# codebits1001/CET-driven-simulation-for-3D-printing-AM-KMC-Approach

Hardware: AMD Instinct MI355X
Metric: kmc_events_per_sec (higher is better)
Workload: dtype f64

## Files before the change

### cet-driven-simulation-for-3d-printing-am-kmc-approach_amd/csrc/kernels.hpp

```cpp
#pragma once
#include "voxel.hpp"
#include "../../include/cetkmc.h"

namespace cetkmc {

struct BlockEnt { double sum; int64_t cnt; };

struct StepState {
    int64_t cur;
    int32_t status;
    int32_t pad0;
    int64_t np_pos;
    int64_t nuc_count;
    double  total;
    int64_t n_events;
    int64_t n_dep;
    double  min_margin;
};

template <class S> __device__ __forceinline__ const auto& ens_rep(unsigned r, const S& sel) { return sel.reps[r]; }
template <class S> __device__ __forceinline__ int ens_rel(const S& sel) { return sel.rel; }
template <class S> __device__ __forceinline__ unsigned ens_nz(const S& sel) { return (unsigned)sel.nz; }
template <class S> __device__ __forceinline__ int64_t ens_stride(const S& sel) { return sel.stride; }
template <class S> __device__ __forceinline__ const long long* ens_offs(const S& sel) { return sel.offs; }
// ... 832 lines not shown
    }
    const int lp = L - 1 - S.gi0;
    if (lp >= 0 && lp < S.nloc)
        for (int64_t idx = gtid; idx < (int64_t)L * L; idx += nthr) {
            const int j = (int)(idx / L), k = (int)(idx - (int64_t)j * L);
            S.dep_val[(int64_t)j * S.pitchT + k] = dep_rate(P, pymax(S.T[S.tidx(lp + 2, j, k)], 1.0));
        }
}

__global__ __launch_bounds__(64) void k_plane_reduce(SlabView S, BlockEnt* __restrict__ blocks,
                                                     const StepState* __restrict__ ss)
{
    if (ss && ss->status) return;
    const int b = blockIdx.x;
    plane_reduce_wave<false>(S.rowsum, S.rowcnt, blocks, S.L, S.Pk, S.gi0, b / 3, b % 3, (int)threadIdx.x);
}

__host__ __device__ __forceinline__ uint64_t mix64(uint64_t x)
{
    x ^= x >> 30; x *= 0xBF58476D1CE4E5B9ULL;
    x ^= x >> 27; x *= 0x94D049BB133111EBULL;
    x ^= x >> 31;
    return x;
}
__host__ __device__ __forceinline__ double counter_uniform(uint64_t seed, uint64_t step, uint64_t site)
{
    uint64_t x = mix64(seed + 0x9E3779B97F4A7C15ULL * (step + 1));
    x = mix64(x ^ (site * 0xD6E8FEB86659FD93ULL + 0x2545F4914F6CDD1DULL));
    return (double)(x >> 11) * (1.0 / 9007199254740992.0);
}
constexpr uint64_t KEY_PICK = 1ull << 40, KEY_THETA = 2ull << 40, KEY_PHI = 3ull << 40, KEY_DEFECT = 4ull << 40,
                   KEY_ACCEPT = 5ull << 40, KEY_DT = 6ull << 40;
__device__ __forceinline__ int dep_species(const KParams& P, double u)
{
    if (u < P.impurity_c) return 3;
    if (u < P.impurity_c + P.impurity_re) return 2;
    return 1;
}

#ifdef CETKMC_SEL_STAMPS
__device__ long long g_sel_stamps[16];
#define SEL_STAMP(q) do { if (threadIdx.x == 0) g_sel_stamps[q] = wall_clock64(); } while (0)
#else
#define SEL_STAMP(q) do { } while (0)
#endif

struct SelCarry {
    double total, u_def, u_th, u_ph;
    double ov[3];
    long long n_events, n_dep, np_pos, cur, nuc_count;
    int ready;
};

struct TreeScratch { double ws[4]; unsigned long long wm[4]; double base; int leaf; };
struct TreeSel { int leaf; double base, total; };
__device__ __forceinline__ double readlane_f64(double v, int lane_uniform)
{
    const int l = __builtin_amdgcn_readfirstlane(lane_uniform);
    return __hiloint2double(__builtin_amdgcn_readlane(__double2hiint(v), l), __builtin_amdgcn_readlane(__double2loint(v), l));
}
template <class RFN>
__device__ __forceinline__ TreeSel tree_select(const double (&lf)[8], unsigned fm, int npt, double base0, RFN rfn, TreeScratch& X, int tid)
{
    const int lane = tid & 63, w = tid >> 6;
    const double p0 = lf[0] + lf[1], p1 = lf[2] + lf[3], p2 = lf[4] + lf[5], p3 = lf[6] + lf[7];
    const double q0 = p0 + p1, q1 = p2 + p3;
    double lv[7];
    lv[0] = q0 + q1;
    lv[1] = lv[0] + dpp_f64(lv[0], 0);
    lv[2] = lv[1] + dpp_f64(lv[1], 1);
    lv[3] = lv[2] + dpp_f64(lv[2], 2);
    lv[4] = lv[3] + dpp_f64(lv[3], 3);
    {
        const unsigned lo = __double2loint(lv[4]), hi = __double2hiint(lv[4]);
        const auto r0 = __builtin_amdgcn_permlane16_swap(lo, lo, false, false);
        const auto r1 = __builtin_amdgcn_permlane16_swap(hi, hi, false, false);
        lv[5] = __hiloint2double((int)r1[0], (int)r0[0]) + __hiloint2double((int)r1[1], (int)r0[1]);
    }
    {
        const unsigned lo = __double2loint(lv[5]), hi = __double2hiint(lv[5]);
        const auto r0 = __builtin_amdgcn_permlane32_swap(lo, lo, false, false);
        const auto r1 = __builtin_amdgcn_permlane32_swap(hi, hi, false, false);
        lv[6] = __hiloint2double((int)r1[0], (int)r0[0]) + __hiloint2double((int)r1[1], (int)r0[1]);
    }
    const unsigned long long mask = __ballot(fm != 0u);
    if (lane == 0) { X.ws[w] = lv[6]; X.wm[w] = mask; }
    __syncthreads();
    const double w0 = X.ws[0], w1 = X.ws[1], w2 = X.ws[2], w3 = X.ws[3];
    const unsigned long long m0 = X.wm[0], m1 = X.wm[1], m2 = X.wm[2], m3 = X.wm[3];
    const double h0 = w0 + w1, h1 = w2 + w3;
    TreeSel out;
    out.total = h0 + h1;
    const double r = rfn(out.total);
    double base = base0;
    int wsel;
    {
        int half;
        if ((m2 | m3) == 0ull || ((m0 | m1) != 0ull && base + h0 >= r)) half = 0;
        else { base += h0; half = 1; }
        const double sl = half ? w2 : w0;
        const unsigned long long ml = half ? m2 : m0, mr = half ? m3 : m1;
        if (mr == 0ull || (ml != 0ull && base + sl >= r)) wsel = 2 * half;
        else { base += sl; wsel = 2 * half + 1; }
    }
    if (w == wsel) {
        int a = 0;
#pragma unroll
        for (int l = 5; l >= 0; --l) {
            const int hw = 1 << l;
            const double sl = readlane_f64(lv[l], a);
            const unsigned long long bits = (hw == 32) ? 0xFFFFFFFFull : ((1ull << hw) - 1ull);
            const bool fl = ((mask >> a) & bits) != 0ull, fr = ((mask >> (a + hw)) & bits) != 0ull;
            if (!(!fr || (fl && base + sl >= r))) { base += sl; a += hw; }
        }
        double bl = base;
        int slot;
        {
            const bool fq0 = (fm & 0x0Fu) != 0u, fq1 = (fm & 0xF0u) != 0u;
            int hq;
            if (!fq1 || (fq0 && bl + q0 >= r)) hq = 0; else { bl += q0; hq = 1; }
            const double pl = hq ? p2 : p0;
            const unsigned f4 = (fm >> (4 * hq)) & 0xFu;
            int hp;
            if ((f4 & 0xCu) == 0u || ((f4 & 0x3u) != 0u && bl + pl >= r)) hp = 0; else { bl += pl; hp = 1; }
            const int s2 = 4 * hq + 2 * hp;
            const double ll = (s2 == 0) ? lf[0] : (s2 == 2) ? lf[2] : (s2 == 4) ? lf[4] : lf[6];
            const unsigned f2 = (fm >> s2) & 0x3u;
            int hl;
            if ((f2 & 0x2u) == 0u || ((f2 & 0x1u) != 0u && bl + ll >= r)) hl = 0; else { bl += ll; hl = 1; }
            slot = s2 + hl;
        }
        const int la = __builtin_amdgcn_readfirstlane(a);
        const int slot_a = __builtin_amdgcn_readlane(slot, la);
        const double base_a = readlane_f64(bl, la);
        if (lane == 0) { X.leaf = (wsel * 64 + la) * npt + slot_a; X.base = base_a; }
    }
    __syncthreads();
    out.leaf = X.leaf; out.base = X.base;
    return out;
}

template <bool IFC>
__device__ __forceinline__ void select_body(const KParams& P, const SlabView* __restrict__ slabs, int nslabs, int L,
                                            int PB, const BlockEnt* __restrict__ blocks, StepState* ss,
                                            const BatchCfg& cfg, const double* __restrict__ u_pick, double r_direct,
                                            const double* __restrict__ ktab_g, cetkmc_event* my_event, int info_only, int ifc_ready,
                                            long long cur_hint = -1, SelCarry* carry = nullptr,
                                            const double* __restrict__ u_defect = nullptr, const double* __restrict__ u_np = nullptr)
{
    __shared__ double leafval[PMAX];
    __shared__ int rowcnt_l[PMAX], voxcnt_l[PMAX];
    __shared__ double ktab[225];
    __shared__ long long red[4];
    __shared__ TreeScratch X;
    __shared__ double sh_u0, sh_base, sh_r;
    __shared__ int sh_go, sh_b, sh_slab;
    __shared__ int sh_gi0[64], sh_nloc[64];
    __shared__ long long sh_ndep;
    const int tid = threadIdx.x;
    SEL_STAMP(0);
    double u0 = 0.0, u_def = 0.0, u_th = 0.0, u_ph = 0.0;
    long long np_pos0 = 0, cur = 0, nuc0 = 0;
    int status0 = 0;
    double margin0 = 1.0;
    if (tid == 0 && cfg.batch) {
        status0 = ss->status;
        margin0 = ss->min_margin;
        np_pos0 = ss->np_pos;
        nuc0 = ss->nuc_count;
        cur = cur_hint >= 0 ? cur_hint : ss->cur;
        if (cfg.rng_mode == 2) {
            const uint64_t g = (uint64_t)(cfg.step0 + cur);
            u0 = counter_uniform(cfg.seed, g, KEY_PICK);
            if (carry) {
                if (cfg.defect_fraction > 0.0) u_def = counter_uniform(cfg.seed, g, KEY_DEFECT);
                u_th = counter_uniform(cfg.seed, g, KEY_THETA); u_ph = counter_uniform(cfg.seed, g, KEY_PHI);
            }
        } else {
            u0 = u_pick[cur];
            if (carry && u_defect && cfg.defect_fraction > 0.0) u_def = u_defect[cur];
            if (carry && u_np && cfg.rng_mode == 1 && np_pos0 + 2 <= cfg.np_cap) { u_th = u_np[np_pos0]; u_ph = u_np[np_pos0 + 1]; }
        }
    }
    if (tid == 0 && carry) carry->ready = 0;
    const SlabView S0 = slabs[0];
    if (tid < nslabs && tid < 64) { sh_gi0[tid] = slabs[tid].gi0; sh_nloc[tid] = slabs[tid].nloc; }
    const int NBk = 3 * L;
    const int npb = PB >= 256 ? (PB >> 8) : 1;
    double lf[8];
    unsigned fm = 0u;
    long long csum = 0;
#pragma unroll
    for (int u = 0; u < 8; ++u) {
        lf[u] = 0.0;
        const int idx = tid * npb + u;
        if (u < npb && idx < NBk) {
            lf[u] = blocks[idx].sum;
            const long long c = blocks[idx].cnt;
            csum += c;
            if (c > 0) fm |= 1u << u;
            if (idx == 3 * (L - 1) + CAT_DEP) sh_ndep = c;
        }
    }
    if (tid < 225) ktab[tid] = ktab_g[tid];
#pragma unroll
    for (int l = 0; l < 6; ++l) csum += __shfl_xor(csum, 1 << l);
    if ((tid & 63) == 0) red[tid >> 6] = csum;
    if (tid == 0) sh_u0 = u0;
    SEL_STAMP(1);
    const TreeSel ta = tree_select(lf, fm, npb, 0.0, [&](double total) { return cfg.batch ? sh_u0 * total : r_direct; }, X, tid);
    SEL_STAMP(2);
    if (tid == 0 && status0) sh_go = 0;
    else if (tid == 0) {
        const double total = ta.total;
        const long long n_events = red[0] + red[1] + red[2] + red[3];
        const long long n_dep = sh_ndep;
        ss->total = total; ss->n_events = n_events; ss->n_dep = n_dep;
        int go = info_only ? 0 : 1;
        if (!info_only) my_event->type = -1;
        const long long dep_draws = (cfg.batch && cfg.rng_mode == 0) ? n_dep : 0;
        if (cfg.batch && go && np_pos0 + dep_draws > cfg.np_cap) {
            ss->status = 2; go = 0;
        } else if (n_events == 0 || total < 1e-25 || !finite_d(total)) {
            if (cfg.batch) { ss->status = 1; ss->np_pos = np_pos0 + dep_draws; }
            go = 0;
        } else if (cfg.batch && go) {
            if (np_pos0 + dep_draws + 2 > cfg.np_cap) { ss->status = 2; go = 0; }
        }
        if (go) {
            const double r = cfg.batch ? u0 * total : r_direct;
            const int b = ta.leaf;
            const int i = b / 3;
            int sl = -1;
            for (int s = 0; s < nslabs; ++s) {
                const int g0 = s < 64 ? sh_gi0[s] : slabs[s].gi0, nl = s < 64 ? sh_nloc[s] : slabs[s].nloc;
                if (i >= g0 && i < g0 + nl) sl = s;
            }
            sh_b = b; sh_slab = sl; sh_base = ta.base; sh_r = r;
            if (sl < 0) go = 0;
            if (go && carry) {
                if (u_np && cfg.rng_mode == 0) { u_th = u_np[np_pos0 + n_dep]; u_ph = u_np[np_pos0 + n_dep + 1]; }
                carry->total = total; carry->n_events = n_events; carry->n_dep = n_dep; carry->np_pos = np_pos0; carry->cur = cur;
                carry->u_def = u_def; carry->u_th = u_th; carry->u_ph = u_ph; carry->nuc_count = nuc0;
                carry->ready = 1;
            }
        }
        sh_go = go;
    }
    __syncthreads();
    SEL_STAMP(3);
    if (!sh_go) return;
    if (carry && tid == 64)
        orient_vec(0.0 + (3.141592653589793 - 0.0) * carry->u_th, 0.0 + (6.283185307179586 - 0.0) * carry->u_ph, carry->ov);
    const SlabView S = (sh_slab == 0) ? S0 : slabs[sh_slab];
    const int b = sh_b, i = b / 3, c = b - 3 * i;
    const int lp = i - S.gi0, li = lp + 2;
    const double r = sh_r;
    const int Pk = S.Pk;
    const int npk = Pk >= 256 ? (Pk >> 8) : 1;
    fm = 0u;
#pragma unroll
    for (int u = 0; u < 8; ++u) {
        lf[u] = 0.0;
        const int idx = tid * npk + u;
        if (u < npk && idx < Pk) {
            int cv = 0;
            if (idx < L) { lf[u] = S.rowsum[((int64_t)lp * 3 + c) * L + idx]; cv = S.rowcnt[((int64_t)lp * 3 + c) * L + idx]; }
            if (cv > 0) fm |= 1u << u;
            rowcnt_l[idx] = cv;
        }
    }
    SEL_STAMP(4);
    const TreeSel tb = tree_select(lf, fm, npk, sh_base, [&](double) { return r; }, X, tid);
    const int j = tb.leaf;
    SEL_STAMP(5);
    fm = 0u;
#pragma unroll
    for (int u = 0; u < 8; ++u) {
        lf[u] = 0.0;
        const int k = tid * npk + u;
        if (u < npk && k < Pk) {
            double sum = 0.0; int cnt = 0;
            int maybe_ifc = 1;
            if (k < L) {
                const int64_t t = S.tidx(li, j, k);
                if (IFC) {
                    const double v_tab = S.vval[t];
                    const unsigned cb = S.cls[S.cidx(li, j, k)];
                    const int c_ifc = (int)(cb >> 2);
                    const bool empty = (cb & 1u) != 0u;
                    maybe_ifc = c_ifc > 0 ? 1 : 0;
                    if (c == CAT_DEP) {
                        const double rate = S.dep_val[(int64_t)j * S.pitchT + k];
                        if (empty && finite_d(rate)) { sum = rate; cnt = 1; }
                    } else if (c == CAT_EMPTY) {
                        if (empty) { sum = v_tab; cnt = c_ifc > 0 ? c_ifc : ((v_tab != 0.0) ? 1 : 0); }
                    } else if (!empty && c_ifc > 0) {
                        sum = v_tab; cnt = c_ifc;
                    }
                } else {
                    const int st = S.state[S.sidx(li, j, k)];
                    const double Traw = S.T[t];
                    auto nb = [&](int mm) -> int { return S.state[S.sidx(li + nbi_rt(mm), j + nbj_rt(mm), k + nbk_rt(mm))]; };
                    auto emit = [&](int cat, int, double rate, int, int) { if (cat == c) { sum += rate; ++cnt; } };
                    eval_voxel(P, S, ktab, li, i, j, k, st, Traw, nb, emit);
                }
            }
            lf[u] = sum;
            if (cnt > 0) fm |= 1u << u;
            leafval[k] = sum;
            voxcnt_l[k] = cnt | (maybe_ifc << 8);
        }
    }
    SEL_STAMP(6);
    const TreeSel tc = tree_select(lf, fm, npk, tb.base, [&](double) { return r; }, X, tid);
    SEL_STAMP(7);
    int rank = 0;
    if (c == CAT_DEP && tid < 64) {
        for (int jj = tid; jj < j; jj += 64) rank += rowcnt_l[jj];
        for (int kk = tid; kk < tc.leaf; kk += 64) rank += voxcnt_l[kk] & 255;
#pragma unroll
        for (int l = 0; l < 6; ++l) rank += __shfl_xor(rank, 1 << l);
    }
    if (tid == 0) {
        const int k = tc.leaf;
        const double base = tc.base;
        int p_type = -1, p_m = -1, p_atom = 0;
        double p_rate = 0.0, p_cum = 0.0;
        const int lc = voxcnt_l[k];
        if ((lc & 255) == 1 && (c == CAT_DEP || (c == CAT_EMPTY && !(lc >> 8)))) {
            p_type = (c == CAT_DEP) ? EV_DEP : EV_NUC;
            p_atom = (c == CAT_DEP) ? 0 : 1;
            p_rate = leafval[k];
            p_cum = base + p_rate;
        } else {
            const int st = S.state[S.sidx(li, j, k)];
            double cum = base;
            bool found = false;
            auto nb = [&](int mm) -> int { return S.state[S.sidx(li + nbi_rt(mm), j + nbj_rt(mm), k + nbk_rt(mm))]; };
            auto emit = [&](int cat, int type, double rate, int m, int atom) {
                if (cat != c || found) return;
                cum += rate;
                p_type = type; p_m = m; p_atom = atom; p_rate = rate;
                p_cum = cum;
                if (cum >= r) found = true;
            };
            eval_voxel(P, S, ktab, li, i, j, k, st, S.T[S.tidx(li, j, k)], nb, emit);
        }
        if (cfg.batch) {
            const double lo = r - (p_cum - p_rate), hi = p_cum - r;
            const double m = (fabs(lo) < fabs(hi) ? fabs(lo) : fabs(hi)) / ta.total;
            if (m < margin0) ss->min_margin = m;
        }
        cetkmc_event ev;
        ev.type = p_type;
        ev.pos[0] = i; ev.pos[1] = j; ev.pos[2] = k;
        ev.target[0] = ev.target[1] = ev.target[2] = -1;
        ev.atom = p_atom; ev.rate = p_rate;
        ev.dep_rank = (p_type == EV_DEP) ? rank : -1;
        ev.theta = 0.0; ev.phi = 0.0;
        if (p_m >= 0) {
            const int di = nbi_rt(p_m), dj = nbj_rt(p_m), dk = nbk_rt(p_m);
            ev.target[0] = i + di; ev.target[1] = j + dj; ev.target[2] = k + dk;
            const int64_t q = (p_type == EV_DIFF) ? S.tidx(li, j, k) : S.tidx(li + di, j + dj, k + dk);
            ev.theta = S.theta[q]; ev.phi = S.phi[q];
        }
        *my_event = ev;
    }
    SEL_STAMP(8);
}

__global__ __launch_bounds__(256) void k_select(KParams P, const SlabView* __restrict__ slabs, int nslabs, int L,
                                                int PB, const BlockEnt* __restrict__ blocks, StepState* ss,
                                                BatchCfg cfg, const double* __restrict__ u_pick, double r_direct,
                                                const double* __restrict__ ktab_g, cetkmc_event* my_event, int info_only, int ifc_ready)
{
    if (ifc_ready) select_body<true>(P, slabs, nslabs, L, PB, blocks, ss, cfg, u_pick, r_direct, ktab_g, my_event, info_only, 1);
    else select_body<false>(P, slabs, nslabs, L, PB, blocks, ss, cfg, u_pick, r_direct, ktab_g, my_event, info_only, 0);
}

__device__ __forceinline__ unsigned ifc_encode(const SlabView& S, int li, int j, int k, bool* interface_out)
{
    const int st = S.state[S.sidx(li, j, k)];
    int sm[14];
#pragma unroll
    for (int m = 0; m < 14; ++m) sm[m] = S.state[S.sidx(li + nbi_rt(m), j + nbj_rt(m), k + nbk_rt(m))];
    unsigned code = 0;
    bool hit = false;
    if (st < 128 && st != 4) {
        code = (unsigned)(st & 3) << 28;
#pragma unroll
        for (int m = 0; m < 14; ++m) {
            unsigned c;
            if (st == 0) { c = (sm[m] >= 1 && sm[m] <= 3) ? (unsigned)sm[m] : 0u; hit |= (c != 0u); }
            else { c = (sm[m] == 0) ? 1u : ((sm[m] != OOB) ? 2u : 0u); hit |= (sm[m] == 0); }
            code |= c << (2 * m);
        }
    } else {
        code = 3u << 30;
    }
    *interface_out = hit;
    return code;
}
__device__ __forceinline__ void ifc_append(const SlabView& S, int lp, int j, int k)
{
    const int64_t t = S.tidx(lp + 2, j, k);
    unsigned* w = reinterpret_cast<unsigned*>(S.ifc_in + (t & ~(int64_t)3));
    const unsigned bit = 1u << (8 * (int)(t & 3));
    if (atomicOr(w, bit) & bit) return;
    const int pos = atomicAdd(S.ifc_n, 1);
    S.ifc_list[pos] = ((unsigned)lp << 20) | ((unsigned)j << 10) | (unsigned)k;
}
__global__ void k_ifc_rebuild(SlabView S)
{
    const int L = S.L;
    const int64_t n = (int64_t)S.nloc * L * L;
    for (int64_t idx = (int64_t)blockIdx.x * blockDim.x + threadIdx.x; idx < n; idx += (int64_t)gridDim.x * blockDim.x) {
        const int k = (int)(idx % L);
        const int64_t t = idx / L;
        const int j = (int)(t % L), lp = (int)(t / L);
        bool hit;
// ... 290 lines not shown
    for (int s = 0; s < nslabs; ++s) {
        const SlabView& S = slabs[s];
        if (wave == 0) {
            if (lane < 16) ifc_touch(P, S, ktab, ev.pos[0], ev.pos[1], ev.pos[2], lane, eval, two, defer);
            else if (two) ifc_touch(P, S, ktab, ev.target[0], ev.target[1], ev.target[2], lane - 16, eval, two, false);
        }
        if (defer && wave == cw) centre_atom_eval(P, S, ev.pos[0], ev.pos[1], ev.pos[2], lane);
    }
}

__device__ __forceinline__ void apply_batch_body(const KParams& P, const SlabView* __restrict__ slabs, int nslabs, int L,
                                                 const cetkmc_event* events_all, int G, StepState* ss,
                                                 const BatchCfg& cfg, const double* __restrict__ u_defect,
                                                 const double* __restrict__ u_np, double* log_total,
                                                 cetkmc_event* log_event, int64_t* log_nev,
                                                 const double* __restrict__ ktab_g, int eval_touched, int* dirty,
                                                 const SelCarry* carry = nullptr)
{
    __shared__ cetkmc_event sh_ev;
    __shared__ int sh_ok;
    SEL_STAMP(9);
    if (threadIdx.x == 0) {
        sh_ok = 0;
        const bool have = carry && carry->ready;
        if (have || (!carry && !ss->status)) {
            cetkmc_event ev;
            ev.type = -1;
            for (int g = 0; g < G; ++g) if (events_all[g].type >= 0) ev = events_all[g];
            const int64_t s = have ? carry->cur : ss->cur;
            if (ev.type < 0) {
                ss->status = 1;
            } else {
                int64_t pos = have ? carry->np_pos : ss->np_pos;
                const int64_t n_dep = have ? carry->n_dep : ss->n_dep;
                if (ev.type == EV_DEP) {
                    const double u = (cfg.rng_mode == 0)
                        ? u_np[pos + ev.dep_rank]
                        : counter_uniform(cfg.seed, (uint64_t)(cfg.step0 + s), (uint64_t)ev.pos[1] * (uint64_t)L + (uint64_t)ev.pos[2]);
                    ev.atom = dep_species(P, u);
                }
                if (cfg.rng_mode == 0) pos += n_dep;
                if (ev.type == EV_DEP || ev.type == EV_NUC) {
                    const uint64_t gs = (uint64_t)(cfg.step0 + s);
                    const double ut = have ? carry->u_th : (cfg.rng_mode == 2 ? counter_uniform(cfg.seed, gs, KEY_THETA) : u_np[pos]);
                    const double up = have ? carry->u_ph : (cfg.rng_mode == 2 ? counter_uniform(cfg.seed, gs, KEY_PHI) : u_np[pos + 1]);
                    ev.theta = 0.0 + (3.141592653589793 - 0.0) * ut;
                    ev.phi = 0.0 + (6.283185307179586 - 0.0) * up;
                    if (cfg.rng_mode != 2) pos += 2;
                    if (ev.type == EV_NUC) { if (have) ss->nuc_count = carry->nuc_count + 1; else ss->nuc_count += 1; }
                }
                const int mk = (cfg.defect_fraction > 0.0 &&
                                (have ? carry->u_def
                                      : (cfg.rng_mode == 2 ? counter_uniform(cfg.seed, (uint64_t)(cfg.step0 + s), KEY_DEFECT) : u_defect[s])) < cfg.defect_fraction) ? 1 : 0;
                apply_event(slabs, nslabs, ev, mk, (have && (ev.type == EV_DEP || ev.type == EV_NUC)) ? carry->ov : nullptr);
                ss->np_pos = pos;
                if (log_total) log_total[s] = have ? carry->total : ss->total;
                if (log_event) log_event[s] = ev;
                if (log_nev) log_nev[s] = have ? carry->n_events : ss->n_events;
                ss->cur = s + 1;
                sh_ev = ev;
                sh_ok = 1;
            }
        }
    }
    SEL_STAMP(10);
    __syncthreads();
    if (sh_ok) apply_touch(P, slabs, nslabs, ktab_g, sh_ev, threadIdx.x, eval_touched, blockDim.x);
    SEL_STAMP(11);
    if (dirty && threadIdx.x == 0) {
        int n = 0;
        if (sh_ok) {
            const int di[11] = {0, 1, 1, -1, -1, 0, 0, 2, -2, 0, 0}, dj[11] = {0, 1, -1, 1, -1, 1, -1, 0, 0, 2, -2};
            for (int v = 0; v < (sh_ev.type == EV_DIFF ? 2 : 1); ++v) {
                const int ci = v ? sh_ev.target[0] : sh_ev.pos[0], cj = v ? sh_ev.target[1] : sh_ev.pos[1];
                for (int q = 0; q < 11; ++q) {
                    const int i = ci + di[q], j = cj + dj[q];
                    if (i < 0 || i >= L || j < 0 || j >= L) continue;
                    const int e = (i << 16) | j;
                    bool dup = false;
                    for (int t = 1; t <= n; ++t) dup |= (dirty[t] == e);
                    if (!dup && n < DIRTY_MAX) dirty[++n] = e;
                }
            }
        }
        dirty[0] = n;
    }
}

__global__ __launch_bounds__(64) void k_apply_batch(KParams P, const SlabView* __restrict__ slabs, int nslabs, int L,
                                                    const cetkmc_event* __restrict__ events_all, int G, StepState* ss,
                                                    BatchCfg cfg, const double* __restrict__ u_defect,
                                                    const double* __restrict__ u_np, double* log_total,
                                                    cetkmc_event* log_event, int64_t* log_nev,
                                                    const double* __restrict__ ktab_g, int eval_touched, int* dirty)
{
    apply_batch_body(P, slabs, nslabs, L, events_all, G, ss, cfg, u_defect, u_np, log_total, log_event, log_nev, ktab_g,
                     eval_touched, dirty);
}
template <bool IFC, class... E>
__global__ __launch_bounds__(256) void k_select_apply(KParams P, const SlabView* __restrict__ slabs, int nslabs, int L,
                                                      int PB, const BlockEnt* __restrict__ blocks, StepState* ss,
                                                      BatchCfg cfg, const double* __restrict__ u_pick,
                                                      const double* __restrict__ ktab_g, cetkmc_event* my_event, int ifc_ready,
                                                      const double* __restrict__ u_defect, const double* __restrict__ u_np,
                                                      double* log_total, cetkmc_event* log_event, int64_t* log_nev,
                                                      int eval_touched, int* dirty, long long cur_hint, E... ens)
{
    if constexpr (sizeof...(E) > 0) {
        const auto& e = ens_rep(blockIdx.x, ens...);
        slabs = &e.view[ens_rel(ens...)]; blocks = e.blocks; ss = e.ss; cfg = e.cfg; u_pick = e.u_pick;
        ktab_g = e.ktab; my_event = e.my_event; u_defect = e.u_defect; u_np = e.u_np;
        log_total = e.log_total; log_event = e.log_event; log_nev = e.log_nev;
    }
    __shared__ cetkmc_event sh_sel;
    __shared__ SelCarry sh_carry;
    (void)my_event;
    if (threadIdx.x == 0) sh_sel.type = -1;
    __syncthreads();
    select_body<IFC>(ens_kp(blockIdx.x, P, ens...), slabs, nslabs, L, PB, blocks, ss, cfg, u_pick, 0.0, ktab_g, &sh_sel, 0, ifc_ready, cur_hint, &sh_carry, u_defect, u_np);
    __syncthreads();
    apply_batch_body(ens_kp(blockIdx.x, P, ens...), slabs, nslabs, L, &sh_sel, 1, ss, cfg, u_defect, u_np, log_total, log_event, log_nev, ktab_g,
                     eval_touched, dirty, &sh_carry);
}

__global__ __launch_bounds__(64) void k_apply_direct(KParams P, const SlabView* __restrict__ slabs, int nslabs, cetkmc_event ev,
                                                     int make_defect, StepState* ss, const double* __restrict__ ktab_g)
{
    if (threadIdx.x == 0) {
        if (ev.type == EV_NUC) ss->nuc_count += 1;
        apply_event(slabs, nslabs, ev, make_defect);
    }
    __syncthreads();
    apply_touch(P, slabs, nslabs, ktab_g, ev, threadIdx.x, 0, blockDim.x);
}

__global__ void k_empty() {}

template <class... E>
__global__ void k_batch_reset(StepState* ss, E... ens)
{
    if constexpr (sizeof...(E) > 0) {
        const auto& e = ens_rep(blockIdx.x, ens...);
        ss = e.ss;
        if (!e.active) { ss->cur = 0; ss->status = 1; ss->np_pos = 0; ss->min_margin = 1.0; return; }
    }
    ss->cur = 0; ss->status = 0; ss->np_pos = 0; ss->min_margin = 1.0;
}

struct ThermalCfg {
    double dt, alpha, inv_dx2, clip_lo, clip_hi, T_nan, rho_cp, latent_coef;
    int laser, use_latent, scrub, ni;
};
struct TableCfg {
    double T_melt, delta_T_c, kT, I0, rate_threshold, K0, nu_dep;
    double* vval;
    double* dep_val;
};
__device__ __forceinline__ double scrub_T(double x, double T_nan, int on)
{
    if (!on) return x;
    if (x != x) return T_nan;
    if (__builtin_isinf(x)) return x > 0 ? 1.7976931348623157e308 : -1.7976931348623157e308;
    return x;
}
__global__ __launch_bounds__(256) void k_thermal(SlabView S, const double* __restrict__ Tin, double* __restrict__ Tout,
                                                 const uint8_t* __restrict__ prev_state, const double* __restrict__ q_top,
                                                 ThermalCfg C, const StepState* __restrict__ ss)
{
    const int L = S.L;
    const int k = blockIdx.x * blockDim.x + threadIdx.x;
    const int j = blockIdx.y, lp = blockIdx.z;
    if (k >= L) return;
    const int li = lp + 2, i = S.gi0 + lp;
// ... 539 lines not shown
```

Before: 15580.

## Run KMC event selection on a single wavefront without block-level syncs

Replaces the 256-thread block tree selection, which staged per-wave sums and masks in shared memory with several __syncthreads, with a single-wavefront select. Each lane now owns up to 32 leaves, reduced with an in-register binary tree and DPP/permlane cross-lane ops. Block, row and voxel picks, counts and deposit ranks are computed inside one wave via readlane, removing the shared rowcnt/voxcnt staging and the barriers around select_body. The cost is more serial work per lane, since one wave handles what four waves used to, plus larger register use from the templated leaf counts.

```diff
diff --git a/cet-driven-simulation-for-3d-printing-am-kmc-approach_amd/csrc/kernels.hpp b/cet-driven-simulation-for-3d-printing-am-kmc-approach_amd/csrc/kernels.hpp
--- a/cet-driven-simulation-for-3d-printing-am-kmc-approach_amd/csrc/kernels.hpp
+++ b/cet-driven-simulation-for-3d-printing-am-kmc-approach_amd/csrc/kernels.hpp
@@ -908,21 +908,41 @@
     int ready;
 };
 
-struct TreeScratch { double ws[4]; unsigned long long wm[4]; double base; int leaf; };
-struct TreeSel { int leaf; double base, total; };
+struct TreeSel { int leaf, lane, slot; double base, total; };
 __device__ __forceinline__ double readlane_f64(double v, int lane_uniform)
 {
     const int l = __builtin_amdgcn_readfirstlane(lane_uniform);
     return __hiloint2double(__builtin_amdgcn_readlane(__double2hiint(v), l), __builtin_amdgcn_readlane(__double2loint(v), l));
 }
-template <class RFN>
-__device__ __forceinline__ TreeSel tree_select(const double (&lf)[8], unsigned fm, int npt, double base0, RFN rfn, TreeScratch& X, int tid)
-{
-    const int lane = tid & 63, w = tid >> 6;
-    const double p0 = lf[0] + lf[1], p1 = lf[2] + lf[3], p2 = lf[4] + lf[5], p3 = lf[6] + lf[7];
-    const double q0 = p0 + p1, q1 = p2 + p3;
+__device__ __forceinline__ double firstlane_f64(double v)
+{
+    return __hiloint2double(__builtin_amdgcn_readfirstlane(__double2hiint(v)), __builtin_amdgcn_readfirstlane(__double2loint(v)));
+}
+template <int NL, class T>
+__device__ __forceinline__ T pick_slot(const T (&x)[NL], int slot)
+{
+    T y[NL];
+#pragma unroll
+    for (int u = 0; u < NL; ++u) y[u] = x[u];
+#pragma unroll
+    for (int d = 0; (NL >> d) > 1; ++d) {
+        const bool odd = ((slot >> d) & 1) != 0;
+#pragma unroll
+        for (int u = 0; u < (NL >> (d + 1)); ++u) y[u] = odd ? y[2 * u + 1] : y[2 * u];
+    }
+    return y[0];
+}
+template <int NL, class RFN>
+__device__ __forceinline__ TreeSel wave_select(const double (&lf)[NL], unsigned fm, double base0, RFN rfn, int lane)
+{
+    static_assert(NL >= 2 && NL <= 32 && (NL & (NL - 1)) == 0, "leaves per lane: a power of two, 2..32");
+    double t[2 * NL];
+#pragma unroll
+    for (int u = 0; u < NL; ++u) t[NL + u] = lf[u];
+#pragma unroll
+    for (int n = NL - 1; n >= 1; --n) t[n] = t[2 * n] + t[2 * n + 1];
     double lv[7];
-    lv[0] = q0 + q1;
+    lv[0] = t[1];
     lv[1] = lv[0] + dpp_f64(lv[0], 0);
     lv[2] = lv[1] + dpp_f64(lv[1], 1);
     lv[3] = lv[2] + dpp_f64(lv[2], 2);
@@ -940,63 +960,171 @@
         lv[6] = __hiloint2double((int)r1[0], (int)r0[0]) + __hiloint2double((int)r1[1], (int)r0[1]);
     }
     const unsigned long long mask = __ballot(fm != 0u);
-    if (lane == 0) { X.ws[w] = lv[6]; X.wm[w] = mask; }
-    __syncthreads();
-    const double w0 = X.ws[0], w1 = X.ws[1], w2 = X.ws[2], w3 = X.ws[3];
-    const unsigned long long m0 = X.wm[0], m1 = X.wm[1], m2 = X.wm[2], m3 = X.wm[3];
-    const double h0 = w0 + w1, h1 = w2 + w3;
     TreeSel out;
-    out.total = h0 + h1;
+    out.total = firstlane_f64(lv[6]);
     const double r = rfn(out.total);
     double base = base0;
-    int wsel;
-    {
-        int half;
-        if ((m2 | m3) == 0ull || ((m0 | m1) != 0ull && base + h0 >= r)) half = 0;
-        else { base += h0; half = 1; }
-        const double sl = half ? w2 : w0;
-        const unsigned long long ml = half ? m2 : m0, mr = half ? m3 : m1;
-        if (mr == 0ull || (ml != 0ull && base + sl >= r)) wsel = 2 * half;
-        else { base += sl; wsel = 2 * half + 1; }
-    }
-    if (w == wsel) {
-        int a = 0;
-#pragma unroll
-        for (int l = 5; l >= 0; --l) {
-            const int hw = 1 << l;
-            const double sl = readlane_f64(lv[l], a);
-            const unsigned long long bits = (hw == 32) ? 0xFFFFFFFFull : ((1ull << hw) - 1ull);
-            const bool fl = ((mask >> a) & bits) != 0ull, fr = ((mask >> (a + hw)) & bits) != 0ull;
-            if (!(!fr || (fl && base + sl >= r))) { base += sl; a += hw; }
-        }
-        double bl = base;
-        int slot;
-        {
-            const bool fq0 = (fm & 0x0Fu) != 0u, fq1 = (fm & 0xF0u) != 0u;
-            int hq;
-            if (!fq1 || (fq0 && bl + q0 >= r)) hq = 0; else { bl += q0; hq = 1; }
-            const double pl = hq ? p2 : p0;
-            const unsigned f4 = (fm >> (4 * hq)) & 0xFu;
-            int hp;
-            if ((f4 & 0xCu) == 0u || ((f4 & 0x3u) != 0u && bl + pl >= r)) hp = 0; else { bl += pl; hp = 1; }
-            const int s2 = 4 * hq + 2 * hp;
-            const double ll = (s2 == 0) ? lf[0] : (s2 == 2) ? lf[2] : (s2 == 4) ? lf[4] : lf[6];
-            const unsigned f2 = (fm >> s2) & 0x3u;
-            int hl;
-            if ((f2 & 0x2u) == 0u || ((f2 & 0x1u) != 0u && bl + ll >= r)) hl = 0; else { bl += ll; hl = 1; }
-            slot = s2 + hl;
-        }
-        const int la = __builtin_amdgcn_readfirstlane(a);
-        const int slot_a = __builtin_amdgcn_readlane(slot, la);
-        const double base_a = readlane_f64(bl, la);
-        if (lane == 0) { X.leaf = (wsel * 64 + la) * npt + slot_a; X.base = base_a; }
-    }
-    __syncthreads();
-    out.leaf = X.leaf; out.base = X.base;
+    int a = 0;
+#pragma unroll
+    for (int l = 5; l >= 0; --l) {
+        const int hw = 1 << l;
+        const double sl = readlane_f64(lv[l], a);
+        const unsigned long long bits = (hw == 32) ? 0xFFFFFFFFull : ((1ull << hw) - 1ull);
+        const bool fl = ((mask >> a) & bits) != 0ull, fr = ((mask >> (a + hw)) & bits) != 0ull;
+        if (!(!fr || (fl && base + sl >= r))) { base += sl; a += hw; }
+    }
+    int n = 1, lo = 0;
+#pragma unroll
+    for (int w = NL / 2; w >= 1; w >>= 1) {
+        double sl = t[2 * (NL / (2 * w))];
+#pragma unroll
+        for (int m = NL / (2 * w) + 1; m < NL / w; ++m) if (n == m) sl = t[2 * m];
+        const unsigned bits = (1u << w) - 1u;
+        const bool fl = ((fm >> lo) & bits) != 0u, fr = ((fm >> (lo + w)) & bits) != 0u;
+        if (!fr || (fl && base + sl >= r)) n = 2 * n;
+        else { base += sl; n = 2 * n + 1; lo += w; }
+    }
+    out.lane = __builtin_amdgcn_readfirstlane(a);
+    out.slot = __builtin_amdgcn_readlane(lo, out.lane);
+    out.base = readlane_f64(base, out.lane);
+    out.leaf = out.lane * NL + out.slot;
     return out;
 }
 
-template <bool IFC>
+struct BlockPick { TreeSel t; long long n_events, n_dep; };
+template <int NL, class RFN>
+__device__ __forceinline__ BlockPick block_pick(const BlockEnt* __restrict__ blocks, int NBk, int dep_blk, RFN rfn, int lane)
+{
+    double lf[NL];
+    unsigned fm = 0u;
+    long long csum = 0, nd = 0;
+#pragma unroll
+    for (int u = 0; u < NL; ++u) {
+        const int idx = lane * NL + u;
+        const bool in = idx < NBk;
+        const BlockEnt be = blocks[in ? idx : NBk - 1];
+        lf[u] = in ? be.sum : 0.0;
+        const long long c = in ? (long long)be.cnt : 0ll;
+        csum += c;
+        if (c > 0) fm |= 1u << u;
+        if (idx == dep_blk) nd = c;
+    }
+    BlockPick o;
+    o.t = wave_select<NL>(lf, fm, 0.0, rfn, lane);
+    o.n_events = (long long)firstlane_f64(wave_tree_sum((double)csum));
+    o.n_dep = (long long)firstlane_f64(wave_tree_sum((double)nd));
+    return o;
+}
+struct RowPick { TreeSel t; int rank; };
+template <int NL>
+__device__ __forceinline__ RowPick row_pick(const SlabView& S, int lp, int c, int L, int Pk, double base0, double r, int lane)
+{
+    double lf[NL];
+    int cv[NL];
+    unsigned fm = 0u;
+#pragma unroll
+    for (int u = 0; u < NL; ++u) {
+        const int idx = lane * NL + u;
+        const bool in = idx < Pk && idx < L;
+        const int64_t q = ((int64_t)lp * 3 + c) * L + (in ? idx : 0);
+        const double v = S.rowsum[q];
+        const int n = S.rowcnt[q];
+        lf[u] = in ? v : 0.0; cv[u] = in ? n : 0;
+        if (cv[u] > 0) fm |= 1u << u;
+    }
+    RowPick o;
+    o.t = wave_select<NL>(lf, fm, base0, [&](double) { return r; }, lane);
+    o.rank = 0;
+    if (c == CAT_DEP) {
+        int s = 0;
+#pragma unroll
+        for (int u = 0; u < NL; ++u) if (lane * NL + u < o.t.leaf) s += cv[u];
+        o.rank = wave_sum_i(s);
+    }
+    return o;
+}
+struct VoxPick { TreeSel t; double val; int lc, rank; };
+template <int NL, bool IFC>
+__device__ __forceinline__ VoxPick voxel_pick(const SlabView& S, int li, int j, int c, int Pk, double base0, double r, int lane,
+                                              const double* leafval, const int* voxcnt_l)
+{
+    const int L = S.L;
+    double lf[NL];
+    int lc[NL];
+    unsigned fm = 0u;
+    if constexpr (IFC) {
+#pragma unroll
+        for (int u = 0; u < NL; ++u) {
+            const int k = lane * NL + u;
+            const bool in = k < Pk && k < L;
+            const int kq = in ? k : 0;
+            const int64_t t = S.tidx(li, j, kq);
+            const double v_tab_l = S.vval[t];
+            const unsigned cb_l = S.cls[S.cidx(li, j, kq)];
+            const double rate_l = c == CAT_DEP ? S.dep_val[(int64_t)j * S.pitchT + kq] : 0.0;
+            double sum = 0.0; int cnt = 0;
+            int maybe_ifc = 1;
+            if (in) {
+                const double v_tab = v_tab_l;
+                const unsigned cb = cb_l;
+                const int c_ifc = (int)(cb >> 2);
+                const bool empty = (cb & 1u) != 0u;
+                maybe_ifc = c_ifc > 0 ? 1 : 0;
+                if (c == CAT_DEP) {
+                    const double rate = rate_l;
+                    if (empty && finite_d(rate)) { sum = rate; cnt = 1; }
+                } else if (c == CAT_EMPTY) {
+                    if (empty) { sum = v_tab; cnt = c_ifc > 0 ? c_ifc : ((v_tab != 0.0) ? 1 : 0); }
+                } else if (!empty && c_ifc > 0) {
+                    sum = v_tab; cnt = c_ifc;
+                }
+            }
+            lf[u] = sum;
+            lc[u] = cnt | (maybe_ifc << 8);
+            if (cnt > 0) fm |= 1u << u;
+        }
+    } else {
+#pragma unroll
+        for (int u = 0; u < NL; ++u) {
+            const int k = lane * NL + u;
+            lf[u] = k < Pk ? leafval[k] : 0.0;
+            lc[u] = k < Pk ? voxcnt_l[k] : (1 << 8);
+            if ((lc[u] & 255) > 0) fm |= 1u << u;
+        }
+    }
+    VoxPick o;
+    o.t = wave_select<NL>(lf, fm, base0, [&](double) { return r; }, lane);
+    o.val = readlane_f64(pick_slot<NL>(lf, o.t.slot), o.t.lane);
+    o.lc = __builtin_amdgcn_readlane(pick_slot<NL>(lc, o.t.slot), o.t.lane);
+    o.rank = 0;
+    if (c == CAT_DEP) {
+        int s = 0;
+#pragma unroll
+        for (int u = 0; u < NL; ++u) if (lane * NL + u < o.t.leaf) s += lc[u] & 255;
+        o.rank = wave_sum_i(s);
+    }
+    return o;
+}
+template <int NLMAX, class F>
+__device__ __forceinline__ auto with_nl(int nl, F f)
+{
+    static_assert(NLMAX == 4 || NLMAX == 8 || NLMAX == 16 || NLMAX == 32, "leaves per lane: 4, 8, 16 or 32");
+    if constexpr (NLMAX == 4) return f(std::integral_constant<int, 4>());
+    else {
+        if (nl <= 4) return f(std::integral_constant<int, 4>());
+        if constexpr (NLMAX == 8) return f(std::integral_constant<int, 8>());
+        else {
+            if (nl == 8) return f(std::integral_constant<int, 8>());
+            if constexpr (NLMAX == 16) return f(std::integral_constant<int, 16>());
+            else {
+                if (nl == 16) return f(std::integral_constant<int, 16>());
+                return f(std::integral_constant<int, 32>());
+            }
+        }
+    }
+}
+
+template <bool IFC, int NLMAX = 32>
 __device__ __forceinline__ void select_body(const KParams& P, const SlabView* __restrict__ slabs, int nslabs, int L,
                                             int PB, const BlockEnt* __restrict__ blocks, StepState* ss,
                                             const BatchCfg& cfg, const double* __restrict__ u_pick, double r_direct,
@@ -1004,225 +1132,178 @@
                                             long long cur_hint = -1, SelCarry* carry = nullptr,
                                             const double* __restrict__ u_defect = nullptr, const double* __restrict__ u_np = nullptr)
 {
-    __shared__ double leafval[PMAX];
-    __shared__ int rowcnt_l[PMAX], voxcnt_l[PMAX];
+    __shared__ double leafval[IFC ? 1 : PMAX];
+    __shared__ int voxcnt_l[IFC ? 1 : PMAX];
     __shared__ double ktab[225];
-    __shared__ long long red[4];
-    __shared__ TreeScratch X;
-    __shared__ double sh_u0, sh_base, sh_r;
-    __shared__ int sh_go, sh_b, sh_slab;
-    __shared__ int sh_gi0[64], sh_nloc[64];
-    __shared__ long long sh_ndep;
-    const int tid = threadIdx.x;
+    __shared__ int sh_go, sh_slab, sh_i, sh_j, sh_c;
+    const int tid = threadIdx.x, lane = tid & 63;
     SEL_STAMP(0);
-    double u0 = 0.0, u_def = 0.0, u_th = 0.0, u_ph = 0.0;
-    long long np_pos0 = 0, cur = 0, nuc0 = 0;
-    int status0 = 0;
-    double margin0 = 1.0;
-    if (tid == 0 && cfg.batch) {
-        status0 = ss->status;
-        margin0 = ss->min_margin;
-        np_pos0 = ss->np_pos;
-        nuc0 = ss->nuc_count;
-        cur = cur_hint >= 0 ? cur_hint : ss->cur;
-        if (cfg.rng_mode == 2) {
-            const uint64_t g = (uint64_t)(cfg.step0 + cur);
-            u0 = counter_uniform(cfg.seed, g, KEY_PICK);
-            if (carry) {
-                if (cfg.defect_fraction > 0.0) u_def = counter_uniform(cfg.seed, g, KEY_DEFECT);
-                u_th = counter_uniform(cfg.seed, g, KEY_THETA); u_ph = counter_uniform(cfg.seed, g, KEY_PHI);
-            }
-        } else {
-            u0 = u_pick[cur];
-            if (carry && u_defect && cfg.defect_fraction > 0.0) u_def = u_defect[cur];
-            if (carry && u_np && cfg.rng_mode == 1 && np_pos0 + 2 <= cfg.np_cap) { u_th = u_np[np_pos0]; u_ph = u_np[np_pos0 + 1]; }
-        }
-    }
-    if (tid == 0 && carry) carry->ready = 0;
-    const SlabView S0 = slabs[0];
-    if (tid < nslabs && tid < 64) { sh_gi0[tid] = slabs[tid].gi0; sh_nloc[tid] = slabs[tid].nloc; }
-    const int NBk = 3 * L;
-    const int npb = PB >= 256 ? (PB >> 8) : 1;
-    double lf[8];
-    unsigned fm = 0u;
-    long long csum = 0;
-#pragma unroll
-    for (int u = 0; u < 8; ++u) {
-        lf[u] = 0.0;
-        const int idx = tid * npb + u;
-        if (u < npb && idx < NBk) {
-            lf[u] = blocks[idx].sum;
-            const long long c = blocks[idx].cnt;
-            csum += c;
-            if (c > 0) fm |= 1u << u;
-            if (idx == 3 * (L - 1) + CAT_DEP) sh_ndep = c;
-        }
-    }
-    if (tid < 225) ktab[tid] = ktab_g[tid];
-#pragma unroll
-    for (int l = 0; l < 6; ++l) csum += __shfl_xor(csum, 1 << l);
-    if ((tid & 63) == 0) red[tid >> 6] = csum;
-    if (tid == 0) sh_u0 = u0;
-    SEL_STAMP(1);
-    const TreeSel ta = tree_select(lf, fm, npb, 0.0, [&](double total) { return cfg.batch ? sh_u0 * total : r_direct; }, X, tid);
-    SEL_STAMP(2);
-    if (tid == 0 && status0) sh_go = 0;
-    else if (tid == 0) {
-        const double total = ta.total;
-        const long long n_events = red[0] + red[1] + red[2] + red[3];
-        const long long n_dep = sh_ndep;
-        ss->total = total; ss->n_events = n_events; ss->n_dep = n_dep;
-        int go = info_only ? 0 : 1;
-        if (!info_only) my_event->type = -1;
-        const long long dep_draws = (cfg.batch && cfg.rng_mode == 0) ? n_dep : 0;
-        if (cfg.batch && go && np_pos0 + dep_draws > cfg.np_cap) {
-            ss->status = 2; go = 0;
-        } else if (n_events == 0 || total < 1e-25 || !finite_d(total)) {
-            if (cfg.batch) { ss->status = 1; ss->np_pos = np_pos0 + dep_draws; }
-            go = 0;
-        } else if (cfg.batch && go) {
-            if (np_pos0 + dep_draws + 2 > cfg.np_cap) { ss->status = 2; go = 0; }
-        }
+    int go = 0, i = 0, j = 0, k = 0, c = 0, li = 0, rank = 0, lc = 0, sl = 0;
+    double r = 0.0, total = 0.0, base = 0.0, leaf_v = 0.0, margin0 = 1.0;
+    SlabView S;
+    if (tid < 64) {
+        double u0 = 0.0;
+        long long np_pos0 = 0;
+        int status0 = 0;
+        if (tid == 0 && cfg.batch) {
+            status0 = ss->status;
+            margin0 = ss->min_margin;
+            np_pos0 = ss->np_pos;
+            const long long cur = cur_hint >= 0 ? cur_hint : ss->cur;
+            if (cfg.rng_mode == 2) u0 = counter_uniform(cfg.seed, (uint64_t)(cfg.step0 + cur), KEY_PICK);
+            else u0 = u_pick[cur];
+        }
+        if (tid == 0 && carry) carry->ready = 0;
+        const SlabView S0 = slabs[0];
+        int g0 = 0, nl = 0;
+        if (lane < nslabs) { g0 = slabs[lane].gi0; nl = slabs[lane].nloc; }
+        const int NBk = 3 * L;
+        const BlockPick bp = with_nl<NLMAX>(PB >= 256 ? (PB >> 6) : 4, [&](auto nlc) {
+            return block_pick<decltype(nlc)::value>(blocks, NBk, 3 * (L - 1) + CAT_DEP, [&](double t) {
+                return cfg.batch ? firstlane_f64(u0) * t : r_direct; }, lane);
+        });
+        total = bp.t.total;
+        SEL_STAMP(1);
+        if (tid == 0 && status0) go = 0;
+        else if (tid == 0) {
+            const long long n_events = bp.n_events, n_dep = bp.n_dep;
+            ss->total = total; ss->n_events = n_events; ss->n_dep = n_dep;
+            go = info_only ? 0 : 1;
+            if (!info_only) my_event->type = -1;
+            const long long dep_draws = (cfg.batch && cfg.rng_mode == 0) ? n_dep : 0;
+            if (cfg.batch && go && np_pos0 + dep_draws > cfg.np_cap) {
+                ss->status = 2; go = 0;
+            } else if (n_events == 0 || total < 1e-25 || !finite_d(total)) {
+                if (cfg.batch) { ss->status = 1; ss->np_pos = np_pos0 + dep_draws; }
+                go = 0;
+            } else if (cfg.batch && go) {
+                if (np_pos0 + dep_draws + 2 > cfg.np_cap) { ss->status = 2; go = 0; }
+            }
+            r = cfg.batch ? u0 * total : r_direct;
+        }
+        go = __builtin_amdgcn_readfirstlane(go);
+        r = firstlane_f64(r);
+        const int b = bp.t.leaf;
+        i = b / 3; c = b - 3 * i;
+        const unsigned long long own = __ballot(lane < nslabs && i >= g0 && i < g0 + nl);
+        sl = own ? 63 - __builtin_clzll(own) : -1;
+        for (int s = 64; s < nslabs; ++s) if (i >= slabs[s].gi0 && i < slabs[s].gi0 + slabs[s].nloc) sl = s;
+        if (sl < 0) go = 0;
+        if (tid == 0 && go && carry) {
+            carry->total = total; carry->n_events = bp.n_events; carry->n_dep = bp.n_dep;
+            carry->ready = 1;
+        }
+        SEL_STAMP(2);
         if (go) {
-            const double r = cfg.batch ? u0 * total : r_direct;
-            const int b = ta.leaf;
-            const int i = b / 3;
-            int sl = -1;
-            for (int s = 0; s < nslabs; ++s) {
-                const int g0 = s < 64 ? sh_gi0[s] : slabs[s].gi0, nl = s < 64 ? sh_nloc[s] : slabs[s].nloc;
-                if (i >= g0 && i < g0 + nl) sl = s;
-            }
-            sh_b = b; sh_slab = sl; sh_base = ta.base; sh_r = r;
-            if (sl < 0) go = 0;
-            if (go && carry) {
-                if (u_np && cfg.rng_mode == 0) { u_th = u_np[np_pos0 + n_dep]; u_ph = u_np[np_pos0 + n_dep + 1]; }
-                carry->total = total; carry->n_events = n_events; carry->n_dep = n_dep; carry->np_pos = np_pos0; carry->cur = cur;
-                carry->u_def = u_def; carry->u_th = u_th; carry->u_ph = u_ph; carry->nuc_count = nuc0;
-                carry->ready = 1;
-            }
-        }
-        sh_go = go;
+            S = (sl == 0) ? S0 : slabs[sl];
+            const int lp = i - S.gi0;
+            li = lp + 2;
+            const int Pk = S.Pk;
+            const int nlk = Pk >= 256 ? (Pk >> 6) : 4;
+            const RowPick rp = with_nl<NLMAX>(nlk, [&](auto nlc) { return row_pick<decltype(nlc)::value>(S, lp, c, L, Pk, bp.t.base, r, lane); });
+            j = rp.t.leaf; base = rp.t.base; rank = rp.rank;
+            SEL_STAMP(3);
+        }
+        if constexpr (!IFC) if (tid == 0) { sh_go = go; sh_slab = sl; sh_i = i; sh_j = j; sh_c = c; }
+    } else {
+        for (int q = tid - 64; q < 225; q += 192) ktab[q] = ktab_g[q];
+        if (carry && tid == 64) {
+            double u_def = 0.0, u_th = 0.0, u_ph = 0.0;
+            long long np_pos0 = 0, cur = 0, nuc0 = 0;
+            if (cfg.batch) {
+                np_pos0 = ss->np_pos;
+                nuc0 = ss->nuc_count;
+                cur = cur_hint >= 0 ? cur_hint : ss->cur;
+                if (cfg.rng_mode == 2) {
+                    const uint64_t g = (uint64_t)(cfg.step0 + cur);
+                    if (cfg.defect_fraction > 0.0) u_def = counter_uniform(cfg.seed, g, KEY_DEFECT);
+                    u_th = counter_uniform(cfg.seed, g, KEY_THETA); u_ph = counter_uniform(cfg.seed, g, KEY_PHI);
+                } else {
+                    if (u_defect && cfg.defect_fraction > 0.0) u_def = u_defect[cur];
+                    if (u_np && cfg.rng_mode == 1 && np_pos0 + 2 <= cfg.np_cap) { u_th = u_np[np_pos0]; u_ph = u_np[np_pos0 + 1]; }
+                    if (u_np && cfg.rng_mode == 0) {
+                        const long long n_dep = blocks[3 * (L - 1) + CAT_DEP].cnt;
+                        if (np_pos0 + n_dep + 2 <= cfg.np_cap) { u_th = u_np[np_pos0 + n_dep]; u_ph = u_np[np_pos0 + n_dep + 1]; }
+                    }
+                }
+            }
+            carry->np_pos = np_pos0; carry->cur = cur; carry->nuc_count = nuc0;
+            carry->u_def = u_def; carry->u_th = u_th; carry->u_ph = u_ph;
+            orient_vec(0.0 + (3.141592653589793 - 0.0) * u_th, 0.0 + (6.283185307179586 - 0.0) * u_ph, carry->ov);
+        }
+    }
+    if constexpr (!IFC) {
+        __syncthreads();
+        if (sh_go) {
+            const SlabView& Sv = slabs[sh_slab];
+            const int iv = sh_i, jv = sh_j, cv = sh_c, liv = iv - Sv.gi0 + 2;
+            for (int kv = tid; kv < Sv.Pk; kv += 256) {
+                double sum = 0.0; int cnt = 0;
+                if (kv < L) {
+                    const int st = Sv.state[Sv.sidx(liv, jv, kv)];
+                    auto nb = [&](int mm) -> int { return Sv.state[Sv.sidx(liv + nbi_rt(mm), jv + nbj_rt(mm), kv + nbk_rt(mm))]; };
+                    auto emit = [&](int cat, int, double rate, int, int) { if (cat == cv) { sum += rate; ++cnt; } };
+                    eval_voxel(P, Sv, ktab, liv, iv, jv, kv, st, Sv.T[Sv.tidx(liv, jv, kv)], nb, emit);
+                }
+                leafval[kv] = sum;
+                voxcnt_l[kv] = cnt | (1 << 8);
+            }
+        }
+        __syncthreads();
+    }
+    if (tid < 64 && go) {
+        const int Pk = S.Pk;
+        const VoxPick vp = with_nl<NLMAX>(Pk >= 256 ? (Pk >> 6) : 4, [&](auto nlc) {
+            return voxel_pick<decltype(nlc)::value, IFC>(S, li, j, c, Pk, base, r, lane, leafval, voxcnt_l); });
+        k = vp.t.leaf; base = vp.t.base; leaf_v = vp.val; lc = vp.lc;
+        rank += vp.rank;
+        SEL_STAMP(4);
     }
     __syncthreads();
-    SEL_STAMP(3);
-    if (!sh_go) return;
-    if (carry && tid == 64)
-        orient_vec(0.0 + (3.141592653589793 - 0.0) * carry->u_th, 0.0 + (6.283185307179586 - 0.0) * carry->u_ph, carry->ov);
-    const SlabView S = (sh_slab == 0) ? S0 : slabs[sh_slab];
-    const int b = sh_b, i = b / 3, c = b - 3 * i;
-    const int lp = i - S.gi0, li = lp + 2;
-    const double r = sh_r;
-    const int Pk = S.Pk;
-    const int npk = Pk >= 256 ? (Pk >> 8) : 1;
-    fm = 0u;
-#pragma unroll
-    for (int u = 0; u < 8; ++u) {
-        lf[u] = 0.0;
-        const int idx = tid * npk + u;
-        if (u < npk && idx < Pk) {
-            int cv = 0;
-            if (idx < L) { lf[u] = S.rowsum[((int64_t)lp * 3 + c) * L + idx]; cv = S.rowcnt[((int64_t)lp * 3 + c) * L + idx]; }
-            if (cv > 0) fm |= 1u << u;
-            rowcnt_l[idx] = cv;
-        }
-    }
-    SEL_STAMP(4);
-    const TreeSel tb = tree_select(lf, fm, npk, sh_base, [&](double) { return r; }, X, tid);
-    const int j = tb.leaf;
     SEL_STAMP(5);
-    fm = 0u;
-#pragma unroll
-    for (int u = 0; u < 8; ++u) {
-        lf[u] = 0.0;
-        const int k = tid * npk + u;
-        if (u < npk && k < Pk) {
-            double sum = 0.0; int cnt = 0;
-            int maybe_ifc = 1;
-            if (k < L) {
-                const int64_t t = S.tidx(li, j, k);
-                if (IFC) {
-                    const double v_tab = S.vval[t];
-                    const unsigned cb = S.cls[S.cidx(li, j, k)];
-                    const int c_ifc = (int)(cb >> 2);
-                    const bool empty = (cb & 1u) != 0u;
-                    maybe_ifc = c_ifc > 0 ? 1 : 0;
-                    if (c == CAT_DEP) {
-                        const double rate = S.dep_val[(int64_t)j * S.pitchT + k];
-                        if (empty && finite_d(rate)) { sum = rate; cnt = 1; }
-                    } else if (c == CAT_EMPTY) {
-                        if (empty) { sum = v_tab; cnt = c_ifc > 0 ? c_ifc : ((v_tab != 0.0) ? 1 : 0); }
-                    } else if (!empty && c_ifc > 0) {
-                        sum = v_tab; cnt = c_ifc;
-                    }
-                } else {
-                    const int st = S.state[S.sidx(li, j, k)];
-                    const double Traw = S.T[t];
-                    auto nb = [&](int mm) -> int { return S.state[S.sidx(li + nbi_rt(mm), j + nbj_rt(mm), k + nbk_rt(mm))]; };
-                    auto emit = [&](int cat, int, double rate, int, int) { if (cat == c) { sum += rate; ++cnt; } };
-                    eval_voxel(P, S, ktab, li, i, j, k, st, Traw, nb, emit);
-                }
-            }
-            lf[u] = sum;
-            if (cnt > 0) fm |= 1u << u;
-            leafval[k] = sum;
-            voxcnt_l[k] = cnt | (maybe_ifc << 8);
-        }
+    if (tid != 0 || !go) return;
+    int p_type = -1, p_m = -1, p_atom = 0;
+    double p_rate = 0.0, p_cum = 0.0;
+    if ((lc & 255) == 1 && (c == CAT_DEP || (c == CAT_EMPTY && !(lc >> 8)))) {
+        p_type = (c == CAT_DEP) ? EV_DEP : EV_NUC;
+        p_atom = (c == CAT_DEP) ? 0 : 1;
+        p_rate = leaf_v;
+        p_cum = base + p_rate;
+    } else {
+        const int st = S.state[S.sidx(li, j, k)];
+        double cum = base;
+        bool found = false;
+        auto nb = [&](int mm) -> int { return S.state[S.sidx(li + nbi_rt(mm), j + nbj_rt(mm), k + nbk_rt(mm))]; };
+        auto emit = [&](int cat, int type, double rate, int m, int atom) {
+            if (cat != c || found) return;
+            cum += rate;
+            p_type = type; p_m = m; p_atom = atom; p_rate = rate;
+            p_cum = cum;
+            if (cum >= r) found = true;
+        };
+        eval_voxel(P, S, ktab, li, i, j, k, st, S.T[S.tidx(li, j, k)], nb, emit);
     }
     SEL_STAMP(6);
-    const TreeSel tc = tree_select(lf, fm, npk, tb.base, [&](double) { return r; }, X, tid);
+    if (cfg.batch) {
+        const double lo = r - (p_cum - p_rate), hi = p_cum - r;
+        const double m = (fabs(lo) < fabs(hi) ? fabs(lo) : fabs(hi)) / total;
+        if (m < margin0) ss->min_margin = m;
+    }
     SEL_STAMP(7);
-    int rank = 0;
-    if (c == CAT_DEP && tid < 64) {
-        for (int jj = tid; jj < j; jj += 64) rank += rowcnt_l[jj];
-        for (int kk = tid; kk < tc.leaf; kk += 64) rank += voxcnt_l[kk] & 255;
-#pragma unroll
-        for (int l = 0; l < 6; ++l) rank += __shfl_xor(rank, 1 << l);
-    }
-    if (tid == 0) {
-        const int k = tc.leaf;
-        const double base = tc.base;
-        int p_type = -1, p_m = -1, p_atom = 0;
-        double p_rate = 0.0, p_cum = 0.0;
-        const int lc = voxcnt_l[k];
-        if ((lc & 255) == 1 && (c == CAT_DEP || (c == CAT_EMPTY && !(lc >> 8)))) {
-            p_type = (c == CAT_DEP) ? EV_DEP : EV_NUC;
-            p_atom = (c == CAT_DEP) ? 0 : 1;
-            p_rate = leafval[k];
-            p_cum = base + p_rate;
-        } else {
-            const int st = S.state[S.sidx(li, j, k)];
-            double cum = base;
-            bool found = false;
-            auto nb = [&](int mm) -> int { return S.state[S.sidx(li + nbi_rt(mm), j + nbj_rt(mm), k + nbk_rt(mm))]; };
-            auto emit = [&](int cat, int type, double rate, int m, int atom) {
-                if (cat != c || found) return;
-                cum += rate;
-                p_type = type; p_m = m; p_atom = atom; p_rate = rate;
-                p_cum = cum;
-                if (cum >= r) found = true;
-            };
-            eval_voxel(P, S, ktab, li, i, j, k, st, S.T[S.tidx(li, j, k)], nb, emit);
-        }
-        if (cfg.batch) {
-            const double lo = r - (p_cum - p_rate), hi = p_cum - r;
-            const double m = (fabs(lo) < fabs(hi) ? fabs(lo) : fabs(hi)) / ta.total;
-            if (m < margin0) ss->min_margin = m;
-        }
-        cetkmc_event ev;
-        ev.type = p_type;
-        ev.pos[0] = i; ev.pos[1] = j; ev.pos[2] = k;
-        ev.target[0] = ev.target[1] = ev.target[2] = -1;
-        ev.atom = p_atom; ev.rate = p_rate;
-        ev.dep_rank = (p_type == EV_DEP) ? rank : -1;
-        ev.theta = 0.0; ev.phi = 0.0;
-        if (p_m >= 0) {
-            const int di = nbi_rt(p_m), dj = nbj_rt(p_m), dk = nbk_rt(p_m);
-            ev.target[0] = i + di; ev.target[1] = j + dj; ev.target[2] = k + dk;
-            const int64_t q = (p_type == EV_DIFF) ? S.tidx(li, j, k) : S.tidx(li + di, j + dj, k + dk);
-            ev.theta = S.theta[q]; ev.phi = S.phi[q];
-        }
-        *my_event = ev;
-    }
+    cetkmc_event ev;
+    ev.type = p_type;
+    ev.pos[0] = i; ev.pos[1] = j; ev.pos[2] = k;
+    ev.target[0] = ev.target[1] = ev.target[2] = -1;
+    ev.atom = p_atom; ev.rate = p_rate;
+    ev.dep_rank = (p_type == EV_DEP) ? rank : -1;
+    ev.theta = 0.0; ev.phi = 0.0;
+    if (p_m >= 0) {
+        const int di = nbi_rt(p_m), dj = nbj_rt(p_m), dk = nbk_rt(p_m);
+        ev.target[0] = i + di; ev.target[1] = j + dj; ev.target[2] = k + dk;
+        const int64_t q = (p_type == EV_DIFF) ? S.tidx(li, j, k) : S.tidx(li + di, j + dj, k + dk);
+        ev.theta = S.theta[q]; ev.phi = S.phi[q];
+    }
+    *my_event = ev;
     SEL_STAMP(8);
 }
 
@@ -1619,6 +1700,7 @@
                 const int mk = (cfg.defect_fraction > 0.0 &&
                                 (have ? carry->u_def
                                       : (cfg.rng_mode == 2 ? counter_uniform(cfg.seed, (uint64_t)(cfg.step0 + s), KEY_DEFECT) : u_defect[s])) < cfg.defect_fraction) ? 1 : 0;
+                SEL_STAMP(15);
                 apply_event(slabs, nslabs, ev, mk, (have && (ev.type == EV_DEP || ev.type == EV_NUC)) ? carry->ov : nullptr);
                 ss->np_pos = pos;
                 if (log_total) log_total[s] = have ? carry->total : ss->total;
@@ -1683,9 +1765,7 @@
     __shared__ SelCarry sh_carry;
     (void)my_event;
     if (threadIdx.x == 0) sh_sel.type = -1;
-    __syncthreads();
-    select_body<IFC>(ens_kp(blockIdx.x, P, ens...), slabs, nslabs, L, PB, blocks, ss, cfg, u_pick, 0.0, ktab_g, &sh_sel, 0, ifc_ready, cur_hint, &sh_carry, u_defect, u_np);
-    __syncthreads();
+    select_body<IFC, (sizeof...(E) > 0) ? 8 : 32>(ens_kp(blockIdx.x, P, ens...), slabs, nslabs, L, PB, blocks, ss, cfg, u_pick, 0.0, ktab_g, &sh_sel, 0, ifc_ready, cur_hint, &sh_carry, u_defect, u_np);
     apply_batch_body(ens_kp(blockIdx.x, P, ens...), slabs, nslabs, L, &sh_sel, 1, ss, cfg, u_defect, u_np, log_total, log_event, log_nev, ktab_g,
                      eval_touched, dirty, &sh_carry);
 }
```

After: 16280 (median of 6 runs). +4.5%, better.
